# intel/QAT-ZSTD-Plugin

Measured on AMD Instinct MI355X. Metric: input MB/s via ZSTD_compress2 L1 128KiB blocks @1/2/4/8 GPU; ratio vs sw zstd, higher is better.
Workload: dtype u8

## Files before the change

### qat-zstd-plugin_amd/csrc/qzstd_kernels.hip

```cpp
#include <hip/hip_runtime.h>

#include <stdint.h>
#include <stdio.h>
#include <stdlib.h>
#include <string.h>

#include <atomic>
#include <mutex>
#include <sched.h>
#include <time.h>
#include <sys/syscall.h>
#include <unistd.h>

#include "qzstd_hip.h"
#include "qzstd_hip_device.h"

#define QZ_PRIO(n) do { if (!CHAIN) __builtin_amdgcn_s_setprio(n); } while (0)

namespace {

constexpr int kMatchWaves = 8;
constexpr int kMatchThreads = kMatchWaves * 64;
constexpr int kThreads = kMatchThreads + 64;
constexpr uint32_t kTileLog = 9;
// ... 328 lines not shown

template <uint32_t W, uint32_t W_END>
__device__ __forceinline__ void parse_windows(const qzstd_hip_profile_t &pf, const Src &src, const uint32_t (&word)[kWin],
                                              uint32_t base, uint32_t n, uint32_t lane, ParseState &st, ParseRecs &r)
{
    if constexpr (W < W_END) {
        parse_window<W>(pf, src, word[W], base, n, lane, st, r);
        parse_windows<W + 1u, W_END>(pf, src, word, base, n, lane, st, r);
    }
}

template <uint32_t W_BEGIN, uint32_t W_END>
__device__ __forceinline__ void parse_tile(const qzstd_hip_profile_t &pf, const Src &src, const uint32_t *pv,
                                           uint32_t *srecOut, uint32_t base, uint32_t n, uint32_t lane, ParseState &st)
{
    uint32_t word[kWin];
#pragma unroll
    for (uint32_t w = W_BEGIN; w < W_END; w++) word[w] = pv[64u * w + lane];
#pragma unroll
    for (uint32_t w = W_BEGIN; w < W_END; w++) asm volatile("" : "+v"(word[w]));
    ParseRecs r = { 0u, 0u, 0u, 0u, 0u, 0u };
    parse_windows<W_BEGIN, W_END>(pf, src, word, base, n, lane, st, r);
    if (lane >= W_BEGIN && lane < W_END) {
        *reinterpret_cast<uint4 *>(srecOut + lane * kSrecWords) = make_uint4(r.r0, r.r1, r.r2, r.r3);
        srecOut[lane * kSrecWords + 4u] = r.r4;
        srecOut[lane * kSrecWords + 5u] = r.r5;
    }
}

struct RepState {
    uint32_t cur, anchor, nseq;
    uint32_t rep1, rep2;
    uint32_t tileSeq;
    uint32_t seg;
};
constexpr uint32_t kRepCap = 32u, kRepMin = 3u;
constexpr uint32_t kLenCapped = 127u;
constexpr uint32_t kChosenBit = 0x80000000u;

__device__ __forceinline__ uint32_t ring_byte(const Src &s, uint32_t x, bool far)
{
    if (far) return reinterpret_cast<const __attribute__((address_space(1))) uint8_t *>(s.g)[x];
    return reinterpret_cast<const __attribute__((address_space(3))) uint8_t *>(s.ring)[x & kRingMask];
}

__device__ __forceinline__ u64 rep_bitmap(const Src &src, uint32_t cur, uint32_t rp, uint32_t n, uint32_t lane, uint32_t ringFrom = 0u)
{
    const uint32_t bpos = cur + lane;
    bool eq = false;
    if (rp != 0u && bpos < n) eq = ring_byte(src, bpos, false) == ring_byte(src, bpos - rp, rp > src.nearLimit || bpos - rp < ringFrom);
    return __ballot(eq);
}

__device__ __forceinline__ u64 rep_record(uint32_t q, uint32_t off, uint32_t L, uint32_t lit)
{
    return (u64)q | ((u64)off << 17) | ((u64)L << 34) | ((u64)lit << 47);
}

__device__ __forceinline__ uint32_t ring_off_s(uint32_t a)
{
    return a & kRingMask;
}

template <bool DEF>
__device__ __forceinline__ void parse_rep_span(const qzstd_hip_profile_t &pf, const Src &src, uint32_t *pvT,
                                               uint32_t base, uint32_t limit, uint32_t n, uint32_t nh, uint32_t lane,
                                               RepState &st, const uint32_t ringFrom = 0u, u64 *recG = nullptr)
{
    const uint32_t segEnd = seg_end(pf, base, n);
    const uint32_t startEnd = segEnd - pf.hashBytes + 1u;
    const uint32_t tileLim = umin(base + kTile, startEnd), stop = umin(limit, startEnd);
    if (st.cur < base) st.cur = base;
    if (st.cur >= stop) return;
    if (pf.segLog && (base >> pf.segLog) != st.seg) {
        st.rep1 = st.rep2 = 0u;
        st.seg = base >> pf.segLog;
    }
    uint32_t rc = rdfirst(ring_off_s(st.cur));
    const __attribute__((address_space(3))) uint8_t *rb = reinterpret_cast<const __attribute__((address_space(3))) uint8_t *>(src.ring);
    while (st.cur < stop) {
        const uint32_t rem = tileLim - st.cur;
        const uint32_t W = umin(pf.repWin, rem), V = umin(W + 2u, rem);
        const uint32_t curIn = st.cur;
        uint32_t wd = 0;
        if (lane < V) wd = pvT[st.cur + lane - base];
        u64 M1, M2;
        if (DEF ? (st.cur - st.rep1 >= ringFrom && st.cur - st.rep2 >= ringFrom)
                : (st.rep1 <= src.nearLimit && st.rep2 <= src.nearLimit)) {
            const uint32_t t1 = rc - st.rep1, t2 = rc - st.rep2;
            const uint32_t r1 = t1 & kRingMask, r2 = t2 & kRingMask;
            const uint32_t A = rb[rc + lane], B1 = rb[r1 + lane], B2 = rb[r2 + lane];
            const u64 in = below(segEnd - st.cur);
            M1 = st.rep1 ? __ballot(A == B1) & in : 0ull;
            M2 = st.rep2 ? __ballot(A == B2) & in : 0ull;
        } else {
            M1 = rep_bitmap(src, st.cur, st.rep1, segEnd, lane, ringFrom);
            M2 = rep_bitmap(src, st.cur, st.rep2, segEnd, lane, ringFrom);
        }
        const uint32_t x1 = __builtin_amdgcn_alignbit((uint32_t)(M1 >> 32), (uint32_t)M1, lane);
        const uint32_t x2 = __builtin_amdgcn_alignbit((uint32_t)(M2 >> 32), (uint32_t)M2, lane);
        const uint32_t rl1 = umin(first_diff_bit(~x1), kRepCap), rl2 = umin(first_diff_bit(~x2), kRepCap);
        const uint32_t rg1 = rl1 < kRepMin ? 0u : (rl1 >= kRepCap ? 1000u : 4u * rl1 + 36u);
        const uint32_t rg2 = rl2 < kRepMin ? 0u : (rl2 >= kRepCap ? 999u : 4u * rl2 + 35u);
        const uint32_t Gh = wd & 0x3FFu;
        const uint32_t G = lane < V ? umax3(Gh, rg1, rg2) : 0u;
        const uint32_t G1 = (uint32_t)__builtin_amdgcn_update_dpp(0, (int)G, 0x130, 0xF, 0xF, true);
        const uint32_t G2 = (uint32_t)__builtin_amdgcn_update_dpp(0, (int)G1, 0x130, 0xF, 0xF, true);
        const bool ok = lane < W && G != 0u && !(G1 > G + 4u) && !(G2 > G + 11u);
        const u64 m = __ballot(ok);
        if (!m) {
            st.cur += W;
            rc = ring_fwd(rc, W);
            continue;
        }
        const uint32_t ks = (uint32_t)__builtin_ctzll(m);
        const uint32_t gh = rdlane(Gh, ks), g1 = rdlane(rg1, ks), g2 = rdlane(rg2, ks);
        const uint32_t q = st.cur + ks;
        uint32_t off, L, from;
        if (g1 <= gh && g2 <= gh) {
            off = rdlane(wd, ks) >> 10;
            L = (gh - 32u + (31u - (uint32_t)__builtin_clz(off + 1u))) >> 2;
            from = pf.capLen;
        } else if (g2 > umax(gh, g1)) {
            off = st.rep2;
            L = rdlane(rl2, ks);
            from = kRepCap;
        } else {
            off = st.rep1;
            L = rdlane(rl1, ks);
            from = kRepCap;
        }
        if (L == from) L = extend_match_from(src, q, off, from, umin(segEnd, ((q >> pf.extLog) + 2u) << pf.extLog), lane,
                                             DEF ? q - off < ringFrom : off > src.nearLimit,
                                             DEF ? (((n + 15u) & ~15u) >> 2) - 1u : 0xFFFFFFFFu);
        if (DEF) {
            if (lane == 0u) recG[st.nseq] = rep_record(q, off, L, q - st.anchor);
        } else if (lane == 0u) {
            uint32_t *r = pvT + (q - base);
            r[0] = kChosenBit | off;
            r[1] = L | ((st.nseq - st.tileSeq) << 17);
            r[2] = st.anchor;
        }
        st.nseq++;
        if (off != st.rep1) {
            st.rep2 = st.rep1;
            st.rep1 = off;
        }
        st.cur = st.anchor = q + L;
        rc = rdfirst(ring_off_s(st.cur));
        (void)curIn;
    }
}

struct PlainParse {
    uint32_t cur, cnt, endA;
};
template <uint32_t W0, uint32_t W1>
__device__ __forceinline__ void parse_plain_windows(const qzstd_hip_profile_t &pf, const Src &src, u64 *recG, const uint32_t base, const uint32_t n,
                                                    const uint32_t lastDw, const uint32_t lane, const uint32_t (&wds)[kWin], PlainParse &st)
{
    u64 smA[kWin], chA[kWin];
    uint32_t lenA[kWin];
#pragma unroll
    for (uint32_t w = W0; w < W1; w++) {
        smA[w] = __ballot((wds[w] & kChosenBit) != 0u);
        lenA[w] = (wds[w] >> 17) & 127u;
    }
#pragma unroll
    for (uint32_t w = W0; w < W1; w++) {
        const uint32_t w0 = base + 64u * w;
        const u64 sm = smA[w];
        uint32_t c = rdfirst(st.cur - w0);
        u64 chosen = 0ull;
        uint32_t lenF = lenA[w];
        uint32_t e = 0u, j = 0u, L = 0u;
        auto chase = [&]() {
            u64 m;
            uint32_t t;
            asm volatile("s_cmp_lt_u32 %[c], 64\n"
                         "s_cbranch_scc0 3f\n"
                         "1:\n"
                         "s_lshr_b64 %[m], %[sm], %[c]\n"
                         "s_cbranch_scc0 2f\n"
                         "s_ff1_i32_b64 %[t], %[m]\n"
                         "s_add_u32 %[j], %[c], %[t]\n"
                         "s_bitset1_b64 %[ch], %[j]\n"
                         "v_readlane_b32 %[L], %[len], %[j]\n"
                         "s_add_u32 %[c], %[j], %[L]\n"
                         "s_cmp_lt_u32 %[c], 64\n"
                         "s_cbranch_scc1 1b\n"
                         "s_mov_b32 %[e], %[c]\n"
                         "s_branch 3f\n"
                         "2:\n"
                         "s_mov_b32 %[e], %[c]\n"
                         "s_movk_i32 %[c], 64\n"
                         "s_mov_b32 %[L], 0\n"
                         "3:\n"
                         : [m] "=&s"(m), [t] "=&s"(t), [j] "+s"(j), [ch] "+s"(chosen), [L] "+s"(L), [c] "+s"(c), [e] "+s"(e)
                         : [sm] "s"(sm), [len] "v"(lenF)
                         : "scc");
        };
        chase();
        while (__builtin_expect(L == kLenCapped, 0)) {
            const uint32_t pj = w0 + j, offj = rdlane(wds[w], j) & 0x1FFFFu;
            L = extend_match_from<true>(src, pj, offj, pf.capLen, umin(seg_end(pf, pj, n), ((pj >> pf.extLog) + 2u) << pf.extLog), lane, true, lastDw);
            if (lane == j) lenF = L;
            c = e = j + L;
            L = 0u;
            chase();
        }
        lenA[w] = lenF;
        st.cur = w0 + c;
        if (chosen) st.endA = w0 + e;
        chA[w] = chosen;
    }
#pragma unroll
    for (uint32_t w = W0; w < W1; w++) {
        const u64 chosen = chA[w];
        const uint32_t rank = __builtin_amdgcn_mbcnt_hi((uint32_t)(chosen >> 32), __builtin_amdgcn_mbcnt_lo((uint32_t)chosen, 0u));
        if ((chosen >> lane) & 1ull) recG[st.cnt + rank] = rep_record(base + 64u * w + lane, wds[w] & 0x1FFFFu, lenA[w], 0u);
        st.cnt += (uint32_t)__popcll(chosen);
    }
}

__device__ __forceinline__ void store_entry(uint4 *out, uint32_t idx, uint32_t off, uint32_t lit, uint32_t ml, uint32_t mark)
{
    if (mark & QZSTD_HIP_MARK_COMPACT)
        reinterpret_cast<u64 *>(out)[idx] = QZSTD_HIP_PACK(off, lit, ml, mark & 0xFFFu);
    else
        out[idx] = make_uint4(off, lit, ml, mark);
}

template <bool REP>
__device__ __forceinline__ void emit_window(const qzstd_hip_profile_t &pf, const Src &src, const uint32_t *srec,
                                            const uint32_t *pvW, uint32_t off, uint32_t len, uint32_t w0, uint32_t rpE,
                                            uint32_t lane, uint4 *out, uint32_t seqCap, uint32_t tileSeq, uint32_t mark)
{
    bool ch;
    uint32_t prevEnd, idx;
    if (REP) {
        const uint32_t r0 = pvW[lane];
        ch = (r0 & kChosenBit) != 0u;
        if (!__ballot(ch)) return;
        const uint32_t r1 = pvW[lane + 1u];
        prevEnd = pvW[lane + 2u];
        off = r0 & 0x1FFFFu;
        len = r1 & 0x1FFFFu;
        idx = tileSeq + (r1 >> 17);
    } else {
        const uint4 rec = *reinterpret_cast<const uint4 *>(srec);
        const u64 chosen = (u64)rec.x | ((u64)rec.y << 32);
        if (!chosen) return;
        const uint32_t anchorIn = rec.z, seqBase = rec.w;
        const uint32_t ext0 = rdfirst(srec[4]);
        if (ext0) {
            const uint32_t ext1 = srec[5];
            if ((ext0 >> 24) == lane) len = ext0 & 0xFFFFFFu;
            if (ext1 && (ext1 >> 24) == lane) len = ext1 & 0xFFFFFFu;
        }
        ch = (chosen >> lane) & 1ull;
        const u64 lower = chosen & below(lane);
        const uint32_t myEnd = w0 + lane + len;
        const int jprev = lower ? 63 - __builtin_clzll(lower) : 0;
        prevEnd = __shfl(myEnd, jprev);
        if (!lower) prevEnd = anchorIn;
        idx = seqBase + __builtin_amdgcn_mbcnt_hi((uint32_t)(chosen >> 32), __builtin_amdgcn_mbcnt_lo((uint32_t)chosen, 0u));
    }
    if (ch) {
        const uint32_t p = w0 + lane, q = p - off;
        const uint32_t lit = p - prevEnd;
        const uint32_t maxb = umin(umin(umin(pf.backExt, lit), q), pf.segLog ? (p & ((1u << pf.segLog) - 1u)) : p);
        uint32_t b = 0;
        if (maxb) {
            const bool far = off > src.nearLimit;
            const uint32_t rp4 = ring_back(rpE, 4u);
            const uint32_t pb = rd32_r(src, p - 4u, rp4, false);
            uint32_t qb;
            if (far) qb = q >= 4u ? rd32u(src, q - 4u, true) : rd32u(src, 0u, true) << (8u * (4u - q));
            else qb = rd32_r(src, q - 4u, ring_back(rp4, off), false);
            const uint32_t x = pb ^ qb;
            b = umin(x ? (uint32_t)__builtin_clz(x) >> 3 : 4u, maxb);
        }
        if (idx < seqCap) store_entry(out, idx, off, lit - b, len + b, mark);
    }
}

__device__ __forceinline__ uint32_t chain_insert_window(uint32_t *tbl, uint32_t st, uint32_t mine, uint32_t lane, bool ordered)
{
    const bool vk = st != kNone;
    const uint32_t slotK = st & 0xFFFFu;
    if (ordered) return vk ? atomicMax(&tbl[slotK], mine) : 0u;
    uint32_t prd = 0u, fin = mine;
    if (vk) {
        uint32_t *e = &tbl[slotK];
        prd = __hip_atomic_load(e, __ATOMIC_RELAXED, __HIP_MEMORY_SCOPE_WORKGROUP);
        atomicMax(e, mine);
        fin = __hip_atomic_load(e, __ATOMIC_RELAXED, __HIP_MEMORY_SCOPE_WORKGROUP);
    }
    u64 rem = __ballot(fin != mine);
    uint32_t predLane = lane;
    while (rem) {
        const uint32_t s0 = rdlane(slotK, (uint32_t)__builtin_ctzll(rem));
        const bool in = vk && slotK == s0;
        const u64 grp = __ballot(in);
        const u64 lower = grp & below(lane);
        if (in && lower) predLane = 63u - (uint32_t)__builtin_clzll(lower);
        rem &= ~grp;
    }
    const uint32_t fromLane = (uint32_t)__shfl((int)mine, (int)predLane);
    return vk ? (predLane != lane ? fromLane : prd) : 0u;
}

__device__ __forceinline__ void chain_insert_tile(const qzstd_hip_profile_t &pf, const Src &src, uint32_t *tbl, uint32_t *P1, uint32_t t0,
                                                  uint32_t n, uint32_t nh, uint32_t lane, bool ordered)
{
    const uint32_t segE = rdfirst(seg_end(pf, t0, n));
    uint32_t stv[kWin];
#pragma unroll
    for (uint32_t k = 0; k < kWin; k++) {
        const uint32_t p = t0 + 64u * k + lane;
        const uint32_t mixH = rd32u(src, p, false) * kPrime1;
        stv[k] = (p < nh && p + 4u <= segE) ? (__umulhi(mixH, pf.tableSize) | (((mixH >> 3) & kTagMask) << 16)) : kNone;
    }
    if (ordered) {
#pragma unroll
        for (uint32_t k = 0; k < kWin; k++) {
            const uint32_t mineK = ((t0 + 64u * k + lane + 1u) << kTagBits) | (stv[k] >> 16);
            uint32_t pred = 0u;
            if (stv[k] != kNone) pred = atomicMax(&tbl[stv[k] & 0xFFFFu], mineK);
            P1[64u * k + lane] = pred;
        }
    } else {
#pragma unroll 1
        for (uint32_t k = 0; k < kWin; k++) {
            const uint32_t st = stv[k];
            const bool vk = st != kNone;
            const uint32_t slotK = st & 0xFFFFu;
            const uint32_t mineK = ((t0 + 64u * k + lane + 1u) << kTagBits) | (st >> 16);
            uint32_t prd = 0u, fin = mineK;
            if (vk) {
                uint32_t *e = &tbl[slotK];
                prd = __hip_atomic_load(e, __ATOMIC_RELAXED, __HIP_MEMORY_SCOPE_WORKGROUP);
                atomicMax(e, mineK);
                fin = __hip_atomic_load(e, __ATOMIC_RELAXED, __HIP_MEMORY_SCOPE_WORKGROUP);
            }
            u64 rem = __ballot(fin != mineK);
            uint32_t predLane = lane;
            while (rem) {
                const uint32_t s0 = rdlane(slotK, (uint32_t)__builtin_ctzll(rem));
                const bool in = vk && slotK == s0;
                const u64 grp = __ballot(in);
                const u64 lower = grp & below(lane);
                if (in && lower) predLane = 63u - (uint32_t)__builtin_clzll(lower);
                rem &= ~grp;
            }
            const uint32_t fromLane = (uint32_t)__shfl((int)mineK, (int)predLane);
            P1[64u * k + lane] = vk ? (predLane != lane ? fromLane : prd) : 0u;
        }
    }
}

struct HistShare {
    uint32_t *flags;
    uint32_t item;
    uint32_t epoch;
    uint32_t spinLimit;
    uint32_t nItems;
    uint32_t *tabFlags;
    uint32_t *linkFlags;
    uint32_t *tabs;
};
constexpr uint32_t kSvcTabStride = QZ_CHAIN_TABLE;
static_assert((uint32_t)kMatchWaves * kPvStride <= QZ_CHAIN_TABLE, "the deferred parse's eight windows of parse words must fit in the head table (QZ_CHAIN_TABLE)");

// ... 624 lines not shown
                        for (int g = 0; g < kG; g++) any = any || m[g];
                        if (any && cl != 0u) {
                            uint32_t v[kG];
#pragma unroll
                            for (int g = 0; g < kG; g++) {
                                m[g] = m[g] && cl < cap;
                                v[g] = 0u;
                                if (m[g]) v[g] = rd32_r(src, q[g] + cl - 3u, ring_fwd(rq[g], cl - 3u), far[g]);
                            }
                            const uint32_t pw = rd32_r(src, p + cl - 3u, ring_fwd(rp, cl - 3u), false);
#pragma unroll
                            for (int g = 0; g < kG; g++) m[g] = m[g] && v[g] == pw;
                        }
                        QZ_CLAP(2)
                        uint32_t Q[kG][5];
#pragma unroll
                        for (int g = 0; g < kG; g++) {
#pragma unroll
                            for (int i = 0; i < 5; i++) Q[g][i] = 0u;
                            if (m[g]) load_dw_r<5>(src, q[g], rq[g], far[g], Q[g]);
                        }
#pragma unroll
                        for (int g = 0; g < kG; g++) {
                            if (m[g] && cl < cap) {
                                uint32_t l = head_cmp(oa, Q[g], q[g] & 3u);
                                if (l == 16u && cap > 16u) l += chunk_len(src, p + 16u, ring_fwd(rp, 16u), p - q[g], far[g]);
                                l = umin(l, cap);
                                const int gn = (int)(4u * l) - (int)(31u - (uint32_t)__builtin_clz(p - q[g] + 1u));
                                if (l >= 4u && (cl == 0u || gn > bg)) { cl = l; off = p - q[g]; bg = gn; }
                            }
                        }
                    }
                    walked += cnt;
                }
                QZ_CLAP(3)
#ifdef QZ_DEBUG_DUMP
                asm volatile("s_waitcnt vmcnt(0)" ::: "memory");
                dC[5] += 1;
#endif
                const bool full = cl != 0u && cl >= cap;
#pragma unroll
                for (uint32_t j = 0; j < kEL; j++) E[j] = full ? 0u : N[j];
                QZ_CLAP(4)
            }
        } else {
        if (TURNS) {
            const uint32_t turn = it * (uint32_t)kMatchWaves + wave;
            uint32_t spins = 0;
            while (__hip_atomic_load(turnCtr, __ATOMIC_ACQUIRE, __HIP_MEMORY_SCOPE_WORKGROUP) != turn && ++spins < (1u << 22))
                __builtin_amdgcn_s_sleep(1);
            if (valid) {
                old = tbl[slot];
                if (validL) oldL = tblL[slotL];
                atomicMax(&tbl[slot], ((p + 1u) << kTagBits) | ((mix >> 3) & kTagMask));
                if (validL) atomicMax(&tblL[slotL], ((p + 1u) << kTagBits) | tagL);
            }
            if (lane == 0u) __hip_atomic_store(turnCtr, turn + 1u, __ATOMIC_RELEASE, __HIP_MEMORY_SCOPE_WORKGROUP);
        }
        if (valid) {
            const uint32_t tag = (mix >> 3) & kTagMask;
            const uint32_t en = pf.nearTab ? nearTab[nslot] : 0xFFFFFFFFu;
            if (!TURNS) {
                atomicMax(&tbl[slot], ((p + 1u) << kTagBits) | tag);
                if (validL) atomicMax(&tblL[slotL], ((p + 1u) << kTagBits) | tagL);
            }
            if (!history) {
            const uint32_t cap = umin(pf.capLen, segE - p);
            uint32_t q1 = kNone, q2 = kNone;
            if (old != 0u && (old & kTagMask) == tag) {
                const uint32_t q = (old >> kTagBits) - 1u;
                if (pf.window == 0u || p - q <= pf.window) q1 = q;
            }
            if (QZ_ABLATED(2u)) q1 = kNone;
            if (QZ_ABLATED(64u) && q1 != kNone && p - q1 > src.nearLimit) q1 = kNone;
            uint32_t l1 = 0, l2 = 0, l3 = 0;
            const bool far1 = q1 != kNone && p - q1 > src.nearLimit;
            if (q1 != kNone) l1 = head_len(src, oa, q1, ring_back(rp, p - q1), far1);
            uint32_t q3 = kNone;
            if (HAS_LONG && validL && oldL != 0u && (oldL & kTagMask) == tagL && !QZ_ABLATED(2u)) q3 = (oldL >> kTagBits) - 1u;
            const bool far3 = q3 != kNone && p - q3 > src.nearLimit;
            if (q3 != kNone) l3 = head_len(src, oa, q3, ring_back(rp, p - q3), far3);
            if (pf.nearTab && (en >> stampShift) == (stamp >> stampShift) && (en & kTagMask) == tag) {
                const uint32_t q = t0 + ((en >> kTagBits) & (kTile - 1u));
                if (q < p && !QZ_ABLATED(2u | 256u)) q2 = q;
            }
            if (q2 != kNone) l2 = head_len(src, oa, q2, ring_back(rp, p - q2), false);
            bool need1 = l1 == 16u && cap > 16u, need2 = l2 == 16u && cap > 16u, need3 = HAS_LONG && l3 == 16u && cap > 16u;
            if (QZ_ABLATED(128u)) need1 = need2 = need3 = false;
            QZ_PRIO(1);
            if (need1 || need2 || need3) {
                const uint32_t rp16 = ring_fwd(rp, 16u);
                uint32_t P[9], pa[8];
                load_dw_r<9>(src, p + 16u, rp16, false, P);
#pragma unroll
                for (int i = 0; i < 8; i++) pa[i] = __builtin_amdgcn_alignbyte(P[i + 1], P[i], p & 3u);
                if (need1) { const uint32_t l = tail_len(src, pa, q1 + 16u, ring_back(rp16, p - q1), far1); l1 = 16u + l; need1 = l == 32u && 48u < cap; }
                if (HAS_LONG && need3) { const uint32_t l = tail_len(src, pa, q3 + 16u, ring_back(rp16, p - q3), far3); l3 = 16u + l; need3 = l == 32u && 48u < cap; }
                if (need2) { const uint32_t l = tail_len(src, pa, q2 + 16u, ring_back(rp16, p - q2), false); l2 = 16u + l; need2 = l == 32u && 48u < cap; }
            }
            while (need1 || need2 || need3) {
                const int which = need1 ? 1 : (need3 ? 3 : 2);
                const uint32_t q = which == 1 ? q1 : (which == 3 ? q3 : q2);
                const uint32_t L = which == 1 ? l1 : (which == 3 ? l3 : l2);
                const uint32_t l = chunk_len(src, p + L, ring_fwd(rp, L), p - q, which == 1 ? far1 : (which == 3 ? far3 : false));
                const bool more = l == 32u && L + 32u < cap;
                if (which == 1) { l1 = L + l; need1 = more; }
                else if (which == 3) { l3 = L + l; need3 = more; }
                else { l2 = L + l; need2 = more; }
            }
            QZ_PRIO(0);
            l1 = umin(l1, cap); l2 = umin(l2, cap); l3 = umin(l3, cap);
            if (l1 >= 4u) { cl = l1; off = p - q1; }
            if (l3 >= 4u && l3 > cl) { cl = l3; off = p - q3; }
            if (l2 >= 4u && l2 >= cl) { cl = l2; off = p - q2; }
            }
        }
        }
        if (!CHAIN && it < nTiles && !history && !QZ_ABLATED(4u)) write_flags(it, cl, off);
#pragma unroll
        for (uint32_t i = kLagT - 1u; i > 0u; i--) { offH[i] = offH[i - 1u]; lenH[i] = lenH[i - 1u]; }
        offH[0] = off;
        lenH[0] = cl;
        rp = ring_fwd(rp, kTile);
        QZ_LAP(dI2)
        if (DEFER && !CHAIN) QZ_BARRIER_LDS(); else __syncthreads();
        QZ_LAP(dW2)
    }
#ifdef QZ_DEBUG_DUMP
    if (!(blk.mark & QZSTD_HIP_MARK_COMPACT)) {
    if (lane == 0) out[blk.seqCap - 3u - wave] = make_uint4((uint32_t)dI1, (uint32_t)dW1, (uint32_t)dI2, (uint32_t)dW2);
    if (lane == 0) out[blk.seqCap - 24u - 2u * wave] = make_uint4((uint32_t)(dC[0] >> 4), (uint32_t)(dC[1] >> 4), (uint32_t)(dC[2] >> 4), (uint32_t)(dC[3] >> 4));
    if (lane == 0) out[blk.seqCap - 25u - 2u * wave] = make_uint4((uint32_t)(dC[4] >> 4), (uint32_t)dC[5], 0u, 0u);
    if (lane == 0) out[blk.seqCap - 12u - wave] = make_uint4(__builtin_amdgcn_s_getreg((4 << 0) | (0 << 6) | (31 << 11)), 0u, 0u, 0u);
    }
#endif
    if constexpr (!DEFER) return 0u;
    }

    if constexpr (DEFER && !REP) {
        constexpr uint32_t kSegLog = 12u, kSeg = 1u << kSegLog, kMaxSegs = QZSTD_HIP_BLOCK_MAX >> kSegLog;
        static_assert(kMaxSegs <= 64u, "one lane per segment in the prefix step");
        constexpr uint32_t kNoAnchor = 0xFFFFFFFFu;
        uint32_t *segCnt = srec, *segEndA = srec + kMaxSegs;
        const uint32_t firstSeg = blk.parseFrom >> kSegLog, nSegs = (nh + kSeg - 1u) >> kSegLog;
#ifdef QZ_DEBUG_DUMP
        const u64 tD0 = __builtin_amdgcn_s_memtime();
#endif
        if (wave == 0u && lane == 0u) segCnt[2u * kMaxSegs] = firstSeg;
        __syncthreads();
#ifdef QZ_DEBUG_DUMP
        const u64 tD1 = __builtin_amdgcn_s_memtime();
#endif
        {
            const uint32_t S0 = rdfirst(segCnt[2u * kMaxSegs]);
            const uint32_t lastDw = (nPad >> 2) - 1u;
            auto load_tile = [&](uint32_t tb, uint32_t (&dst)[kWin]) {
#pragma unroll
                for (uint32_t j = 0; j < kWin; j++) dst[j] = p1B[tb + 64u * j + lane];
            };
            uint32_t nxt[kWin];
            uint32_t sgN = S0 + wave;
            if (sgN < nSegs) load_tile(sgN << kSegLog, nxt);
            while (sgN < nSegs) {
                const uint32_t sg = sgN;
                sgN = sg + (uint32_t)kMatchWaves;
                const uint32_t segStart = sg << kSegLog;
                u64 *recG = reinterpret_cast<u64 *>(p1B + segStart);
                const uint32_t tEnd = umin(segStart + kSeg, nTiles << kTileLog);
                PlainParse st = { segStart, 0u, kNoAnchor };
                for (uint32_t base = segStart; base < tEnd; base += kTile) {
                    uint32_t wds[kWin];
#pragma unroll
                    for (uint32_t j = 0; j < kWin; j++) wds[j] = nxt[j];
                    const uint32_t nb = base + kTile < tEnd ? base + kTile : sgN << kSegLog;
                    if (base + kTile < tEnd || sgN < nSegs) load_tile(nb, nxt);
                    parse_plain_windows<0, kWin>(pf, src, recG, base, n, lastDw, lane, wds, st);
                }
                if (lane == 0u) { segCnt[sg] = st.cnt; segEndA[sg] = st.endA; }
            }
        }
#ifdef QZ_DEBUG_DUMP
        const u64 tD2 = __builtin_amdgcn_s_memtime();
#endif
        __syncthreads();
#ifdef QZ_DEBUG_DUMP
        const u64 tD3 = __builtin_amdgcn_s_memtime();
#endif
        const bool mine = lane >= firstSeg && lane < nSegs;
        const uint32_t cv = mine ? segCnt[lane] : 0u, ev = mine ? segEndA[lane] : kNoAnchor;
        uint32_t incl = cv, last = ev;
#pragma unroll
        for (uint32_t d = 1; d < kMaxSegs; d <<= 1) {
            const uint32_t ci = (uint32_t)__shfl_up((int)incl, d), li = (uint32_t)__shfl_up((int)last, d);
            if (lane >= d) { incl += ci; if (last == kNoAnchor) last = li; }
        }
        const uint32_t total = rdlane(incl, kMaxSegs - 1u), lastAll = rdlane(last, kMaxSegs - 1u);
        const uint32_t anchorEndAll = lastAll == kNoAnchor ? blk.parseFrom : lastAll;
        {
            for (uint32_t sg = firstSeg + wave; sg < nSegs; sg += (uint32_t)kMatchWaves) {
                const u64 *recG = reinterpret_cast<const u64 *>(p1B + (sg << kSegLog));
                const uint32_t cnt = rdlane(cv, sg), first = rdlane(incl, sg) - cnt;
                uint32_t anchorIn = blk.parseFrom;
                if (sg > 0u) { const uint32_t a = rdlane(last, sg - 1u); if (a != kNoAnchor) anchorIn = a; }
                constexpr uint32_t kU = 4u;
                for (uint32_t k0 = 0; k0 < cnt; k0 += 64u * kU) {
                    u64 r[kU], rp1[kU];
#pragma unroll
                    for (uint32_t u = 0; u < kU; u++) {
                        const uint32_t k = k0 + 64u * u + lane;
                        r[u] = k < cnt ? recG[k] : 0ull;
                        rp1[u] = (k < cnt && k) ? recG[k - 1u] : 0ull;
                    }
                    uint32_t P0[kU], P1[kU], Q0[kU], Q1[kU], lit[kU], maxb[kU];
#pragma unroll
                    for (uint32_t u = 0; u < kU; u++) {
                        const uint32_t k = k0 + 64u * u + lane;
                        const uint32_t pm = (uint32_t)r[u] & 0x1FFFFu, off = (uint32_t)(r[u] >> 17) & 0x1FFFFu;
                        lit[u] = k ? pm - (((uint32_t)rp1[u] & 0x1FFFFu) + ((uint32_t)(rp1[u] >> 34) & 0x1FFFu))
                                   : pm - anchorIn;
                        const uint32_t q = pm - off;
                        maxb[u] = k < cnt ? umin(umin(umin(pf.backExt, lit[u]), q), pm & (kSeg - 1u)) : 0u;
                        P0[u] = P1[u] = Q0[u] = Q1[u] = 0u;
                        if (maxb[u]) {
                            const uint32_t pa = pm >= 4u ? pm - 4u : 0u, qa = q >= 4u ? q - 4u : 0u;
                            P0[u] = src.g[pa >> 2]; P1[u] = src.g[(pa >> 2) + 1u];
                            Q0[u] = src.g[qa >> 2]; Q1[u] = src.g[(qa >> 2) + 1u];
                        }
                    }
#pragma unroll
                    for (uint32_t u = 0; u < kU; u++) {
                        const uint32_t k = k0 + 64u * u + lane;
                        if (k < cnt) {
                            const uint32_t pm = (uint32_t)r[u] & 0x1FFFFu, off = (uint32_t)(r[u] >> 17) & 0x1FFFFu, len = (uint32_t)(r[u] >> 34) & 0x1FFFu;
                            const uint32_t q = pm - off;
                            uint32_t b = 0;
                            if (maxb[u]) {
                                const uint32_t pa = pm >= 4u ? pm - 4u : 0u, qa = q >= 4u ? q - 4u : 0u;
                                uint32_t pb = __builtin_amdgcn_alignbyte(P1[u], P0[u], pa & 3u), qb = __builtin_amdgcn_alignbyte(Q1[u], Q0[u], qa & 3u);
                                if (pm < 4u) pb <<= 8u * (4u - pm);
                                if (q < 4u) qb <<= 8u * (4u - q);
                                const uint32_t x = pb ^ qb;
                                b = umin(x ? (uint32_t)__builtin_clz(x) >> 3 : 4u, maxb[u]);
                            }
                            const uint32_t idx = first + k;
                            if (idx < blk.seqCap) store_entry(out, idx, off, lit[u] - b, len + b, blk.mark);
                        }
                    }
                }
            }
#ifdef QZ_DEBUG_DUMP
            if (lane == 0 && !(blk.mark & QZSTD_HIP_MARK_COMPACT))
                out[blk.seqCap - 44u - wave] = make_uint4((uint32_t)(tD1 - tD0), (uint32_t)(tD2 - tD1), (uint32_t)(tD3 - tD2), (uint32_t)(__builtin_amdgcn_s_memtime() - tD3));
#endif
        }
        if (wave != 0u) return 0u;
        uint32_t count = total + 1u;
        if (lane == 0 && total < blk.seqCap) store_entry(out, total, 0u, n - anchorEndAll, 0u, blk.mark);
        if (count >= blk.seqCap - 1u) count = QZSTD_HIP_NSEQ_ERROR;
        return count;
    }

    if constexpr (DEFER && REP) {
        constexpr uint32_t kSegLog = 12u, kSeg = 1u << kSegLog, kSegsPerQ = kRing >> kSegLog;
        static_assert(kSegsPerQ == (uint32_t)kMatchWaves, "one wave per segment of a quarter");
        constexpr uint32_t kNoAnchor = 0xFFFFFFFFu;
        __syncthreads();
        uint32_t *pvW = tbl + wave * kPvStride;
        uint32_t *ctl = srec;
        const uint32_t firstSeg = blk.parseFrom >> kSegLog, nSegs = (nh + kSeg - 1u) >> kSegLog;
        uint32_t total = 0u, anchorCarry = blk.parseFrom;
        for (uint32_t Q = firstSeg / kSegsPerQ; Q * kSegsPerQ < nSegs; Q++) {
            const uint32_t qs = Q * kRing;
            for (uint32_t o = qs + tid * 16u; o < umin(qs + kRing, nPad); o += (uint32_t)kMatchThreads * 16u) {
                const uint4 v = g128[o >> 4];
                ring128[(o & kRingMask) >> 4] = v;
                if ((o & kRingMask) < kMirror) ring128[(kRing + (o & kRingMask)) >> 4] = v;
            }
            __syncthreads();
            const uint32_t sg = Q * kSegsPerQ + wave;
            const uint32_t segStart = sg << kSegLog;
            u64 *recG = reinterpret_cast<u64 *>(p1B + segStart);
            uint32_t cnt = 0u, endA = kNoAnchor;
            if (sg >= firstSeg && sg < nSegs) {
                const uint32_t tEnd = umin(segStart + kSeg, nTiles << kTileLog);
                uint32_t nxt[kWin];
#pragma unroll
                for (uint32_t j = 0; j < kWin; j++) nxt[j] = p1B[segStart + 64u * j + lane];
                {
                    RepState st = { segStart, segStart, 0u, 0u, 0u, 0u, sg };
                    for (uint32_t base = segStart; base < tEnd; base += kTile) {
#pragma unroll
                        for (uint32_t j = 0; j < kWin; j++) pvW[64u * j + lane] = nxt[j];
                        if (base + kTile < tEnd) {
#pragma unroll
                            for (uint32_t j = 0; j < kWin; j++) nxt[j] = p1B[base + kTile + 64u * j + lane];
                        }
                        parse_rep_span<true>(pf, src, pvW, base, base + kTile, n, nh, lane, st, qs, recG);
                    }
                    cnt = st.nseq;
                    if (cnt) endA = st.anchor;
                }
            }
            if (lane == 0u) { ctl[wave] = cnt; ctl[kSegsPerQ + wave] = endA; }
            __syncthreads();
            {
                const uint32_t cv = lane < 2u * kSegsPerQ ? ctl[lane] : 0u;
                uint32_t before = 0u, all = 0u, anchorIn = anchorCarry, anchorOut = anchorCarry;
#pragma unroll
                for (uint32_t j = 0; j < kSegsPerQ; j++) {
                    const uint32_t c = rdlane(cv, j), a = rdlane(cv, kSegsPerQ + j);
                    if (j < wave) { before += c; if (a != kNoAnchor) anchorIn = a; }
                    all += c;
                    if (a != kNoAnchor) anchorOut = a;
                }
                const uint32_t cnt = rdlane(cv, wave);
                for (uint32_t k0 = 0; k0 < cnt; k0 += 64u) {
                    const uint32_t k = k0 + lane;
                    if (k < cnt) {
                        const u64 r = recG[k];
                        const uint32_t pm = (uint32_t)r & 0x1FFFFu, off = (uint32_t)(r >> 17) & 0x1FFFFu, len = (uint32_t)(r >> 34) & 0x1FFFu;
                        uint32_t lit = pm - anchorIn;
                        if (k) lit = (uint32_t)(r >> 47) & 0x1FFFu;
                        const uint32_t q = pm - off;
                        const uint32_t maxb = umin(umin(umin(pf.backExt, lit), q), pm & (kSeg - 1u));
                        uint32_t b = 0;
                        if (maxb) {
                            const uint32_t pb = rd32u(src, pm - 4u, false);
                            uint32_t qb;
                            if (q < qs + 4u) qb = q >= 4u ? rd32u(src, q - 4u, true) : rd32u(src, 0u, true) << (8u * (4u - q));
                            else qb = rd32u(src, q - 4u, false);
                            const uint32_t x = pb ^ qb;
                            b = umin(x ? (uint32_t)__builtin_clz(x) >> 3 : 4u, maxb);
                        }
                        const uint32_t idx = total + before + k;
                        if (idx < blk.seqCap) store_entry(out, idx, off, lit - b, len + b, blk.mark);
                    }
                }
                total += all;
                anchorCarry = anchorOut;
            }
            __syncthreads();
        }
        if (wave != 0u) return 0u;
        uint32_t count = total + 1u;
        if (lane == 0 && total < blk.seqCap) store_entry(out, total, 0u, n - anchorCarry, 0u, blk.mark);
        if (count >= blk.seqCap - 1u) count = QZSTD_HIP_NSEQ_ERROR;
        return count;
    }
    return 0u;
}

#ifndef QZ_WAVES_PER_EU
#define QZ_WAVES_PER_EU 5
#endif
#define QZ_OCCUPANCY __attribute__((amdgpu_waves_per_eu(QZ_WAVES_PER_EU)))
template <bool HAS_LONG, bool REP, bool CHAIN, bool TURNS, bool NEAR>
__global__ __launch_bounds__(kThreads) QZ_OCCUPANCY void qzstd_find_sequences_kernel(LaunchArgs args)
{
    const qzstd_hip_block_t blk = args.blocks[blockIdx.x];
    const uint32_t count = qz_item<HAS_LONG, REP, CHAIN, TURNS, NEAR, true>(args, blk, args.src + blk.srcOff, args.seqs + blk.seqOff,
                                                              CHAIN ? args.chain + (size_t)blockIdx.x * args.chainStride : nullptr,
                                                              reinterpret_cast<uint32_t *>(args.chain + (size_t)blockIdx.x * args.chainStride + args.chainEntries),
                                                              HistShare{ nullptr, 0u, 0u, 0u, 0u, nullptr, nullptr, nullptr });
    asm volatile("s_waitcnt vmcnt(0)" ::: "memory");
    __syncthreads();
    if (threadIdx.x == 0u)
        __hip_atomic_store(args.nseq + blockIdx.x, count, __ATOMIC_RELEASE, __HIP_MEMORY_SCOPE_SYSTEM);
}

constexpr uint32_t kSvcQueue = 4096u;
constexpr uint32_t kSvcRing = 256u;
constexpr uint32_t kSvcMaxItems = 32u;
constexpr uint32_t kSvcSlots = 1024u;
constexpr uint32_t kSvcRejected = 0xFFFFFFFEu;

struct SvcDev {
    u64 items[kSvcQueue][8];
    uint32_t head;
    uint32_t done;
    uint32_t quit;
    uint32_t spinFails;
    uint32_t started;
    uint32_t taken;
    uint32_t pad[2];
    uint32_t sliceFlag[kSvcSlots][kSvcMaxItems];
    uint32_t histFlag[kSvcSlots][kSvcMaxItems];
    uint32_t tabFlag[kSvcSlots][kSvcMaxItems];
    uint32_t linkFlag[kSvcSlots][kSvcMaxItems];
};

struct SvcHost {
    u64 ring[kSvcRing][8];
    uint32_t state;
    uint32_t quitReq;
    u64 consumed;
    u64 itemsDone;
    uint32_t spinFails;
    uint32_t pad;
    u64 dbg[8];
};

typedef __attribute__((address_space(1))) u64 *gu64p;
typedef __attribute__((address_space(1))) uint32_t *gu32p;

__device__ __forceinline__ u64 svc_tag(u64 n, uint32_t entries) { return (n / entries) % 255ull + 1ull; }
__device__ __forceinline__ u64 svc_payload(u64 g) { return g & 0x00FFFFFFFFFFFFFFull; }


constexpr uint32_t kSvcProfiles = 24u;
__device__ __forceinline__ uint32_t svc_profile_index(uint32_t levelByte) { return ((levelByte & 0x7Fu) - 1u) + ((levelByte & 0x80u) ? 12u : 0u); }

template <bool HAS_LONG, bool REP, bool CHAIN, bool TURNS, bool MULTI>
__global__ __launch_bounds__(kThreads) void qzstd_service_worker(LaunchArgs args, SvcDev *sv, uint32_t ctlOff, uint32_t spinLimit, const qzstd_hip_profile_t *profs)
{
    const uint32_t tid = threadIdx.x, lane = tid & 63u;
    const uint32_t wave = rdfirst(tid >> 6);
    uint32_t *ctl = (uint32_t *)(__attribute__((address_space(3))) uint32_t *)(size_t)(kLdsBase + ctlOff);
    if (tid == 0u) (void)__hip_atomic_fetch_add(&sv->started, 1u, QZ_RLX_AGENT);
    for (;;) {
        if (wave == 0u) {
            uint32_t t = 0u;
            if (lane == 0u) t = __hip_atomic_fetch_add(&sv->head, 1u, QZ_RLX_AGENT);
            t = rdfirst(t);
            const u64 want = svc_tag(t, kSvcQueue);
            const u64 *slot = sv->items[t & (kSvcQueue - 1u)];
            u64 g = 0;
            uint32_t got = 0u;
            for (;;) {
                if (lane < 8u) g = __hip_atomic_load(slot + lane, QZ_RLX_AGENT);
                else if (lane == 8u) g = (u64)__hip_atomic_load(&sv->quit, QZ_RLX_AGENT);
                const bool mine = lane >= 8u || (g >> 56) == want;
                if (__all(mine)) { got = 1u; break; }
                if (rdlane((uint32_t)g, 8u) != 0u) break;
                __builtin_amdgcn_s_sleep(4);
            }
            if (lane < 8u) { ctl[2u * lane] = (uint32_t)g; ctl[2u * lane + 1u] = (uint32_t)(svc_payload(g) >> 32); }
            if (lane == 8u) ctl[16] = got;
            if (lane == 0u && got) (void)__hip_atomic_fetch_add(&sv->taken, 1u, QZ_RLX_AGENT);
        }
        __syncthreads();
        if (rdfirst(ctl[16]) == 0u) return;
        const u64 q0 = rdfirst(ctl[0]) | ((u64)rdfirst(ctl[1]) << 32), q1 = rdfirst(ctl[2]) | ((u64)rdfirst(ctl[3]) << 32),
                  q2 = rdfirst(ctl[4]) | ((u64)rdfirst(ctl[5]) << 32), q3 = rdfirst(ctl[6]) | ((u64)rdfirst(ctl[7]) << 32),
                  q4 = rdfirst(ctl[8]) | ((u64)rdfirst(ctl[9]) << 32), q5 = rdfirst(ctl[10]), q6 = rdfirst(ctl[12]),
                  q7 = rdfirst(ctl[14]) | ((u64)rdfirst(ctl[15]) << 32);
        const uint8_t *hSrc = (const uint8_t *)q0;
        uint8_t *dSrc = (uint8_t *)q1;
        uint4 *out = (uint4 *)q2;
        uint32_t *countWord = (uint32_t *)q3;
        qzstd_hip_block_t blk;
        blk.srcOff = 0; blk.seqOff = 0;
        blk.srcLen = (uint32_t)q4 & 0x3FFFFu;
        blk.parseFrom = (uint32_t)(q4 >> 18) & 0x3FFFFu;
        blk.seqCap = (uint32_t)q5 & 0xFFFFFFu;
        const uint32_t nItemsReq = (uint32_t)(q5 >> 24) & 63u;
        const uint32_t k = (uint32_t)(q4 >> 36) & 63u, slotIdx = (uint32_t)(q4 >> 42) & (kSvcSlots - 1u);
        const uint32_t epoch = (uint32_t)q6 & 0xFFFFFFu;
        blk.mark = epoch;
        {
            const uint32_t end = (blk.srcLen + 15u) & ~15u;
            if (wave == 0u) {
                uint32_t spins = 0u, okS = 1u;
                while (__hip_atomic_load(countWord, QZ_RLX_SYSTEM) == QZSTD_HIP_NSEQ_STAGING) {
                    if (++spins > spinLimit) { okS = 0u; break; }
                    __builtin_amdgcn_s_sleep(8);
                }
                __builtin_amdgcn_fence(__ATOMIC_ACQUIRE, "");
                if (lane == 0u) ctl[18] = okS;
            }
            __syncthreads();
            const bool staged = rdfirst(ctl[18]) != 0u;
            for (uint32_t o = blk.parseFrom + tid * 16u; o < end && staged; o += (uint32_t)kThreads * 16u) {
                const u64 a = __hip_atomic_load((const u64 *)(hSrc + o), QZ_RLX_SYSTEM);
                const u64 b = __hip_atomic_load((const u64 *)(hSrc + o + 8u), QZ_RLX_SYSTEM);
                __hip_atomic_store((u64 *)(dSrc + o), a, QZ_RLX_AGENT);
                __hip_atomic_store((u64 *)(dSrc + o + 8u), b, QZ_RLX_AGENT);
            }
            asm volatile("s_waitcnt vmcnt(0)" ::: "memory");
            __syncthreads();
            if (wave == 0u) {
                if (lane == 0u && staged) __hip_atomic_store(&sv->sliceFlag[slotIdx][k], epoch, QZ_RLX_AGENT);
                uint32_t spins = 0u, ok = 1u;
                for (;;) {
                    const bool there = lane >= k || __hip_atomic_load(&sv->sliceFlag[slotIdx][lane], QZ_RLX_AGENT) == epoch;
                    if (__all(there)) break;
                    if (++spins > spinLimit) { ok = 0u; break; }
                    __builtin_amdgcn_s_sleep(2);
                }
                __builtin_amdgcn_fence(__ATOMIC_ACQUIRE, "agent");
                if (lane == 0u) ctl[17] = staged ? ok : 0u;
            }
            __syncthreads();
        }
        uint32_t count = QZSTD_HIP_NSEQ_ERROR;
#define QZ_SVC_ITEM(A, L, R, C, T)                                                                                                            \
    qz_item<L, R, C, T, false>(A, blk, dSrc, out, (C) ? (uint4 *)q7 : nullptr, (C) ? (uint32_t *)(q7 + (u64)QZSTD_HIP_BLOCK_MAX * (8ull * QZSTD_HIP_CHAIN_ENTRY_LINKS)) : nullptr, \
                               HistShare{ (C) ? &sv->histFlag[slotIdx][0] : nullptr, k, epoch, spinLimit, nItemsReq, &sv->tabFlag[slotIdx][0],   \
                                          &sv->linkFlag[slotIdx][0], (C) ? (uint32_t *)(q7 + (u64)QZSTD_HIP_BLOCK_MAX * (8ull * QZSTD_HIP_CHAIN_ENTRY_LINKS + 4ull)) : nullptr })
        if (rdfirst(ctl[17]) != 0u) {
            if (MULTI) {
                LaunchArgs a2 = args;
                const uint32_t pi = rdfirst(svc_profile_index((uint32_t)(q6 >> 24) & 0xFFu));
                a2.prof = profs[pi < kSvcProfiles ? pi : 0u];
                const bool chain = a2.prof.chainDepth != 0u, rpt = a2.prof.repWin != 0u, turns = a2.prof.subTileLog != 0u;
                if (chain) count = rpt ? QZ_SVC_ITEM(a2, false, true, true, true) : QZ_SVC_ITEM(a2, false, false, true, true);
                else if (turns) count = rpt ? QZ_SVC_ITEM(a2, false, true, false, true) : QZ_SVC_ITEM(a2, false, false, false, true);
                else count = rpt ? QZ_SVC_ITEM(a2, false, true, false, false) : QZ_SVC_ITEM(a2, false, false, false, false);
            } else {
// ... 1255 lines not shown
```

Before: 23940.

## Parse two segments per wave in the deferred plain parse

Each match wave now parses two independent 4KiB segments at once, interleaving their scalar match-chasing chains in one inline asm loop so each serial dependency chain has independent work to hide its latency. Tile prefetching is doubled to keep both segments' next words loaded. This adds register pressure, which the static asserts check against the waves-per-EU budget, and lengthens the loop body. Block edge cases depend on a round-count assumption that the asserts only partly enforce.

```diff
diff --git a/qat-zstd-plugin_amd/csrc/qzstd_kernels.hip b/qat-zstd-plugin_amd/csrc/qzstd_kernels.hip
--- a/qat-zstd-plugin_amd/csrc/qzstd_kernels.hip
+++ b/qat-zstd-plugin_amd/csrc/qzstd_kernels.hip
@@ -504,74 +504,116 @@
     }
 }
 
+#ifndef QZ_WAVES_PER_EU
+#define QZ_WAVES_PER_EU 5
+#endif
+#define QZ_OCCUPANCY __attribute__((amdgpu_waves_per_eu(QZ_WAVES_PER_EU)))
+
 struct PlainParse {
     uint32_t cur, cnt, endA;
 };
 template <uint32_t W0, uint32_t W1>
-__device__ __forceinline__ void parse_plain_windows(const qzstd_hip_profile_t &pf, const Src &src, u64 *recG, const uint32_t base, const uint32_t n,
-                                                    const uint32_t lastDw, const uint32_t lane, const uint32_t (&wds)[kWin], PlainParse &st)
-{
-    u64 smA[kWin], chA[kWin];
-    uint32_t lenA[kWin];
+__device__ __forceinline__ void parse_plain_windows2(const qzstd_hip_profile_t &pf, const Src &src, u64 *recGA, u64 *recGB, const uint32_t baseA,
+                                                     const uint32_t baseB, const uint32_t n, const uint32_t lastDw, const uint32_t lane,
+                                                     const uint32_t (&wdsA)[kWin], const uint32_t (&wdsB)[kWin], PlainParse &stA, PlainParse &stB)
+{
+    u64 smA[kWin], smB[kWin], chA[kWin], chB[kWin];
+    uint32_t lenA[kWin], lenB[kWin];
 #pragma unroll
     for (uint32_t w = W0; w < W1; w++) {
-        smA[w] = __ballot((wds[w] & kChosenBit) != 0u);
-        lenA[w] = (wds[w] >> 17) & 127u;
+        smA[w] = __ballot((wdsA[w] & kChosenBit) != 0u);
+        smB[w] = __ballot((wdsB[w] & kChosenBit) != 0u);
+        lenA[w] = (wdsA[w] >> 17) & 127u;
+        lenB[w] = (wdsB[w] >> 17) & 127u;
     }
 #pragma unroll
     for (uint32_t w = W0; w < W1; w++) {
-        const uint32_t w0 = base + 64u * w;
-        const u64 sm = smA[w];
-        uint32_t c = rdfirst(st.cur - w0);
-        u64 chosen = 0ull;
-        uint32_t lenF = lenA[w];
-        uint32_t e = 0u, j = 0u, L = 0u;
+        const uint32_t w0A = baseA + 64u * w, w0B = baseB + 64u * w;
+        const uint32_t cInA = rdfirst(stA.cur - w0A), cInB = rdfirst(stB.cur - w0B);
+        const bool liveA = cInA < 64u && (smA[w] >> (cInA & 63u)) != 0ull, liveB = cInB < 64u && (smB[w] >> (cInB & 63u)) != 0ull;
+        u64 rA = liveA ? smA[w] : 0ull, rB = liveB ? smB[w] : 0ull;
+        uint32_t cA = cInA, cB = cInB;
+        u64 chosenA = 0ull, chosenB = 0ull, extA = 0ull, extB = 0ull;
+        uint32_t lenFA = lenA[w], lenFB = lenB[w];
+        uint32_t jA = 0u, jB = 0u, LA = 0u, LB = 0u;
         auto chase = [&]() {
-            u64 m;
-            uint32_t t;
-            asm volatile("s_cmp_lt_u32 %[c], 64\n"
-                         "s_cbranch_scc0 3f\n"
+            u64 mA, mB, x;
+            uint32_t tA, tB;
+            asm volatile("s_lshr_b64 %[mA], %[rA], %[cA]\n"
+                         "s_lshr_b64 %[mB], %[rB], %[cB]\n"
+                         "s_or_b64 %[x], %[mA], %[mB]\n"
+                         "s_cbranch_scc0 2f\n"
                          "1:\n"
-                         "s_lshr_b64 %[m], %[sm], %[c]\n"
-                         "s_cbranch_scc0 2f\n"
-                         "s_ff1_i32_b64 %[t], %[m]\n"
-                         "s_add_u32 %[j], %[c], %[t]\n"
-                         "s_bitset1_b64 %[ch], %[j]\n"
-                         "v_readlane_b32 %[L], %[len], %[j]\n"
-                         "s_add_u32 %[c], %[j], %[L]\n"
-                         "s_cmp_lt_u32 %[c], 64\n"
+                         "s_ff1_i32_b64 %[tA], %[mA]\n"
+                         "s_ff1_i32_b64 %[tB], %[mB]\n"
+                         "s_add_u32 %[tA], %[cA], %[tA]\n"
+                         "s_add_u32 %[tB], %[cB], %[tB]\n"
+                         "s_cmp_lg_u64 %[mA], 0\n"
+                         "s_cselect_b32 %[jA], %[tA], %[jA]\n"
+                         "s_cmp_lg_u64 %[mB], 0\n"
+                         "s_cselect_b32 %[jB], %[tB], %[jB]\n"
+                         "s_bitset1_b64 %[chA], %[jA]\n"
+                         "s_bitset1_b64 %[chB], %[jB]\n"
+                         "v_readlane_b32 %[LA], %[lenA], %[jA]\n"
+                         "v_readlane_b32 %[LB], %[lenB], %[jB]\n"
+                         "s_add_u32 %[cA], %[jA], %[LA]\n"
+                         "s_add_u32 %[cB], %[jB], %[LB]\n"
+                         "s_cmp_lt_u32 %[cA], 64\n"
+                         "s_cselect_b64 %[rA], %[rA], 0\n"
+                         "s_cmp_lt_u32 %[cB], 64\n"
+                         "s_cselect_b64 %[rB], %[rB], 0\n"
+                         "s_lshr_b64 %[mA], %[rA], %[cA]\n"
+                         "s_lshr_b64 %[mB], %[rB], %[cB]\n"
+                         "s_or_b64 %[x], %[mA], %[mB]\n"
                          "s_cbranch_scc1 1b\n"
-                         "s_mov_b32 %[e], %[c]\n"
-                         "s_branch 3f\n"
                          "2:\n"
-                         "s_mov_b32 %[e], %[c]\n"
-                         "s_movk_i32 %[c], 64\n"
-                         "s_mov_b32 %[L], 0\n"
-                         "3:\n"
-                         : [m] "=&s"(m), [t] "=&s"(t), [j] "+s"(j), [ch] "+s"(chosen), [L] "+s"(L), [c] "+s"(c), [e] "+s"(e)
-                         : [sm] "s"(sm), [len] "v"(lenF)
+                         : [mA] "=&s"(mA), [mB] "=&s"(mB), [x] "=&s"(x), [tA] "=&s"(tA), [tB] "=&s"(tB), [jA] "+s"(jA), [jB] "+s"(jB),
+                           [chA] "+s"(chosenA), [chB] "+s"(chosenB), [LA] "+s"(LA), [LB] "+s"(LB), [cA] "+s"(cA), [cB] "+s"(cB), [rA] "+s"(rA),
+                           [rB] "+s"(rB)
+                         : [lenA] "v"(lenFA), [lenB] "v"(lenFB)
                          : "scc");
         };
         chase();
-        while (__builtin_expect(L == kLenCapped, 0)) {
-            const uint32_t pj = w0 + j, offj = rdlane(wds[w], j) & 0x1FFFFu;
-            L = extend_match_from<true>(src, pj, offj, pf.capLen, umin(seg_end(pf, pj, n), ((pj >> pf.extLog) + 2u) << pf.extLog), lane, true, lastDw);
-            if (lane == j) lenF = L;
-            c = e = j + L;
-            L = 0u;
+        for (;;) {
+            if (__builtin_expect(umax(LA, LB) < kLenCapped, 1)) break;
+            const bool capA = liveA && LA == kLenCapped && !((extA >> jA) & 1ull), capB = liveB && LB == kLenCapped && !((extB >> jB) & 1ull);
+            if (__builtin_expect(!(capA || capB), 1)) break;
+            if (capA) {
+                const uint32_t pj = w0A + jA, offj = rdlane(wdsA[w], jA) & 0x1FFFFu;
+                const uint32_t L = extend_match_from<true>(src, pj, offj, pf.capLen, umin(seg_end(pf, pj, n), ((pj >> pf.extLog) + 2u) << pf.extLog), lane, true, lastDw);
+                if (lane == jA) lenFA = L;
+                extA |= 1ull << jA;
+                cA = jA + L;
+                rA = cA < 64u ? smA[w] : 0ull;
+            }
+            if (capB) {
+                const uint32_t pj = w0B + jB, offj = rdlane(wdsB[w], jB) & 0x1FFFFu;
+                const uint32_t L = extend_match_from<true>(src, pj, offj, pf.capLen, umin(seg_end(pf, pj, n), ((pj >> pf.extLog) + 2u) << pf.extLog), lane, true, lastDw);
+                if (lane == jB) lenFB = L;
+                extB |= 1ull << jB;
+                cB = jB + L;
+                rB = cB < 64u ? smB[w] : 0ull;
+            }
             chase();
         }
-        lenA[w] = lenF;
-        st.cur = w0 + c;
-        if (chosen) st.endA = w0 + e;
-        chA[w] = chosen;
+        lenA[w] = lenFA;
+        lenB[w] = lenFB;
+        if (liveA) stA.endA = w0A + cA;
+        if (liveB) stB.endA = w0B + cB;
+        stA.cur = w0A + (liveA ? umax(cA, 64u) : umax(cInA, 64u));
+        stB.cur = w0B + (liveB ? umax(cB, 64u) : umax(cInB, 64u));
+        chA[w] = liveA ? chosenA : 0ull;
+        chB[w] = liveB ? chosenB : 0ull;
     }
 #pragma unroll
     for (uint32_t w = W0; w < W1; w++) {
-        const u64 chosen = chA[w];
-        const uint32_t rank = __builtin_amdgcn_mbcnt_hi((uint32_t)(chosen >> 32), __builtin_amdgcn_mbcnt_lo((uint32_t)chosen, 0u));
-        if ((chosen >> lane) & 1ull) recG[st.cnt + rank] = rep_record(base + 64u * w + lane, wds[w] & 0x1FFFFu, lenA[w], 0u);
-        st.cnt += (uint32_t)__popcll(chosen);
+        const u64 cA = chA[w], cB = chB[w];
+        const uint32_t rankA = __builtin_amdgcn_mbcnt_hi((uint32_t)(cA >> 32), __builtin_amdgcn_mbcnt_lo((uint32_t)cA, 0u));
+        const uint32_t rankB = __builtin_amdgcn_mbcnt_hi((uint32_t)(cB >> 32), __builtin_amdgcn_mbcnt_lo((uint32_t)cB, 0u));
+        if ((cA >> lane) & 1ull) recGA[stA.cnt + rankA] = rep_record(baseA + 64u * w + lane, wdsA[w] & 0x1FFFFu, lenA[w], 0u);
+        if ((cB >> lane) & 1ull) recGB[stB.cnt + rankB] = rep_record(baseB + 64u * w + lane, wdsB[w] & 0x1FFFFu, lenB[w], 0u);
+        stA.cnt += (uint32_t)__popcll(cA);
+        stB.cnt += (uint32_t)__popcll(cB);
     }
 }
 
@@ -1502,31 +1544,44 @@
         const u64 tD1 = __builtin_amdgcn_s_memtime();
 #endif
         {
+            constexpr uint32_t kParseSegs = 2u;
+            static_assert(kMaxSegs % ((uint32_t)kMatchWaves * kParseSegs) == 0u, "a full block is whole rounds of waves x segments in flight (a shorter one, or one parsed from a later segment on, ends in a ragged round: B is not there)");
+            static_assert(kParseSegs * 3u * kWin <= 512u / QZ_WAVES_PER_EU - 32u, "the segments in flight x (words + prefetched words + lengths) per lane must leave 32 of the VGPRs that QZ_WAVES_PER_EU allows a wave");
             const uint32_t S0 = rdfirst(segCnt[2u * kMaxSegs]);
-            const uint32_t lastDw = (nPad >> 2) - 1u;
+            const uint32_t lastDw = (nPad >> 2) - 1u, posEnd = nTiles << kTileLog;
             auto load_tile = [&](uint32_t tb, uint32_t (&dst)[kWin]) {
 #pragma unroll
                 for (uint32_t j = 0; j < kWin; j++) dst[j] = p1B[tb + 64u * j + lane];
             };
-            uint32_t nxt[kWin];
+            uint32_t nxtA[kWin] = {}, nxtB[kWin] = {};
             uint32_t sgN = S0 + wave;
-            if (sgN < nSegs) load_tile(sgN << kSegLog, nxt);
+            if (sgN < nSegs) load_tile(sgN << kSegLog, nxtA);
+            if (sgN + (uint32_t)kMatchWaves < nSegs) load_tile((sgN + (uint32_t)kMatchWaves) << kSegLog, nxtB);
             while (sgN < nSegs) {
-                const uint32_t sg = sgN;
-                sgN = sg + (uint32_t)kMatchWaves;
-                const uint32_t segStart = sg << kSegLog;
-                u64 *recG = reinterpret_cast<u64 *>(p1B + segStart);
-                const uint32_t tEnd = umin(segStart + kSeg, nTiles << kTileLog);
-                PlainParse st = { segStart, 0u, kNoAnchor };
-                for (uint32_t base = segStart; base < tEnd; base += kTile) {
-                    uint32_t wds[kWin];
-#pragma unroll
-                    for (uint32_t j = 0; j < kWin; j++) wds[j] = nxt[j];
-                    const uint32_t nb = base + kTile < tEnd ? base + kTile : sgN << kSegLog;
-                    if (base + kTile < tEnd || sgN < nSegs) load_tile(nb, nxt);
-                    parse_plain_windows<0, kWin>(pf, src, recG, base, n, lastDw, lane, wds, st);
+                const uint32_t sgA = sgN, sgB = sgN + (uint32_t)kMatchWaves;
+                sgN = sgA + kParseSegs * (uint32_t)kMatchWaves;
+                const uint32_t startA = sgA << kSegLog, startB = sgB << kSegLog;
+                u64 *recGA = reinterpret_cast<u64 *>(p1B + startA), *recGB = reinterpret_cast<u64 *>(p1B + startB);
+                const uint32_t endA = umin(startA + kSeg, posEnd), endB = sgB < nSegs ? umin(startB + kSeg, posEnd) : startB;
+                PlainParse stA = { startA, 0u, kNoAnchor }, stB = { startB, 0u, kNoAnchor };
+                for (uint32_t t = 0; startA + t < endA; t += kTile) {
+                    const uint32_t baseA = startA + t, baseB = startB + t;
+                    const bool hasB = baseB < endB;
+                    uint32_t wdsA[kWin], wdsB[kWin];
+#pragma unroll
+                    for (uint32_t j = 0; j < kWin; j++) { wdsA[j] = nxtA[j]; wdsB[j] = hasB ? nxtB[j] : 0u; }
+                    const bool moreA = baseA + kTile < endA;
+                    if (moreA) load_tile(baseA + kTile, nxtA);
+                    else if (sgN < nSegs) load_tile(sgN << kSegLog, nxtA);
+                    if (moreA) { if (baseB + kTile < endB) load_tile(baseB + kTile, nxtB); }
+                    else if (sgN + (uint32_t)kMatchWaves < nSegs) load_tile((sgN + (uint32_t)kMatchWaves) << kSegLog, nxtB);
+                    parse_plain_windows2<0, kWin / 2u>(pf, src, recGA, recGB, baseA, baseB, n, lastDw, lane, wdsA, wdsB, stA, stB);
+                    parse_plain_windows2<kWin / 2u, kWin>(pf, src, recGA, recGB, baseA, baseB, n, lastDw, lane, wdsA, wdsB, stA, stB);
                 }
-                if (lane == 0u) { segCnt[sg] = st.cnt; segEndA[sg] = st.endA; }
+                if (lane == 0u) {
+                    segCnt[sgA] = stA.cnt; segEndA[sgA] = stA.endA;
+                    if (sgB < nSegs) { segCnt[sgB] = stB.cnt; segEndA[sgB] = stB.endA; }
+                }
             }
         }
 #ifdef QZ_DEBUG_DUMP
@@ -1700,10 +1755,6 @@
     return 0u;
 }
 
-#ifndef QZ_WAVES_PER_EU
-#define QZ_WAVES_PER_EU 5
-#endif
-#define QZ_OCCUPANCY __attribute__((amdgpu_waves_per_eu(QZ_WAVES_PER_EU)))
 template <bool HAS_LONG, bool REP, bool CHAIN, bool TURNS, bool NEAR>
 __global__ __launch_bounds__(kThreads) QZ_OCCUPANCY void qzstd_find_sequences_kernel(LaunchArgs args)
 {
```

Measured after the change: 22380. 6.5% lower.
